# jhauret/vibravox

Hardware: AMD Instinct MI355X
Metric: EBEN train-step audio-seconds/sec (gen+disc) (higher is better)
Workload: dtype bf16

## Files before the change

### vibravox_amd/csrc/tap3.h

```cpp
#pragma once
#include "common.h"

namespace eben {

typedef unsigned u32x4 __attribute__((ext_vector_type(4)));

struct Tap3Args {
  const float* x; const float* xmask; const u32x4* wp; const int* tab;
  const float* bias; const float* res; const float* emask; float* y;
  int B, G, Cg, Mg, Cx, Cy, Lx, Ly;
  int S, OS, dstep, J0, mode, off0, nt, nph;
  int ps_pad, ps_k, ps_d, ps_kstep;
  int reflect, accumulate, in_mode;
  int res_rows, em_seg, em_map[4];
  const float* fm_sums; float fm_gs;
  float in_slope, out_slope, res_slope, emask_slope;
  int CI_T, CI_B, CP, ncc, PLEN, CSTRIDE, nxb;
  unsigned s_magic;
  int ntt, nmt, tab_phase;
  long long w_tile, w_phase;
  const u32x4* xh; const u32x4* xl;
  uint2* yh; uint2* yl;
  const uint2* eh; const uint2* el;
  const unsigned* ec;
  int CBx, CBy, bl_ref_off, bl_pad;
  int pr_S, pr_cbg, pr_Ly, pr_order;
  unsigned xq, xr;
  unsigned m_nph, m_ntt, m_B, m_nmt;
  int id_fast, pg_n;
  int big_XT, big_PPT, big_tiles;
  unsigned m_cstride, m_plen;
  struct PG { int J, off0, minoff, nt, oo, span; unsigned span_magic; int pad; } pg[8];
};

struct Tap3Plan {
  int ok;
  int mode, G, Cg, Mg, S, OS, dstep, kstep, nph, J, Lx, Ly, Cx, Cy, off0, nt, ps_pad;
  int FM, BM, BN, WCHU;
  int dense;
  int npw, npx, KSC;
  int CI_T, CI_B, CP, ncc, PLEN, CSTRIDE, nxbuf, XRB;
  int nmt, ntt, NCH, tab_phase;
  long long w_tile, w_phase, tab_off_floats;
  size_t packed_floats, lds_bytes;
  int big, WM, WN, TM, TN, RING, XT, PPT, xbuf_stride;
};

int tap4_launch(const Tap3Plan& p, const Tap3Args& a, hipStream_t st);

}
```

### vibravox_amd/csrc/tapconv3.hip

```cpp
#include "common.h"
#include "tap3.h"

#include <cstdlib>

namespace eben {

typedef float f32x16 __attribute__((ext_vector_type(16)));
typedef float f32x2 __attribute__((ext_vector_type(2)));
typedef __bf16 bf16x8 __attribute__((ext_vector_type(8)));
typedef __bf16 bf16x2 __attribute__((ext_vector_type(2)));

__device__ __forceinline__ unsigned pack_bf16(float a, float b) {
  const f32x2 v = {a, b};
  return __builtin_bit_cast(unsigned, __builtin_convertvector(v, bf16x2));
}

#ifndef EBEN_T3_KSC
#define EBEN_T3_KSC 4
#endif
#ifndef EBEN_T3_DBG
#define EBEN_T3_DBG 0
#endif
#if EBEN_T3_DBG & 512
constexpr int T3_STAMP_ROWS = 65536;
// ... 1059 lines not shown
  const int wave = __builtin_amdgcn_readfirstlane(tid >> 6);
  const int k = P.k;
  const int NCP = P.ncc * P.CP;
  int item = blockIdx.x;
  const int col = item % NCP; item /= NCP;
  const int fm = item % P.FM; item /= P.FM;
  const int mt = item % P.nmt;
  const int g = item / P.nmt;
  const int cc = col / P.CP, cp = col - cc * P.CP;
  const int m0 = mt * P.BM + fm * 32;
  const int c0 = cc * P.CI_T + 16 * cp;
  const int nrow = P.Mg - m0 < 32 ? P.Mg - m0 : 32;
  const int nch = P.Cg - c0 < 16 ? P.Cg - c0 : 16;
  const int RS = (P.mode == 0 ? 16 : 32) * k | 1;
  if (nrow > 0 && nch > 0) {
    const int nlines = P.mode == 0 ? nrow : nch;
    const int run = (P.mode == 0 ? nch : nrow) * k;
    for (int ln = wave; ln < nlines; ln += 4) {
      const long long src = P.mode == 0 ? ((long long)(g * P.Cout_g + m0 + ln) * P.Cin_g + c0) * k
                                        : ((long long)(g * P.Cout_g + c0 + ln) * P.Cin_g + m0) * k;
      const float sc = P.scale ? P.scale[g * P.Cout_g + (P.mode == 0 ? m0 : c0) + ln] : 1.f;
      for (int i = lane; i < run; i += 64) p3c[ln * RS + i] = P.w[src + i] * sc;
    }
  }
  __syncthreads();
  const int r = lane & 31, h = lane >> 5;
  const bool row_ok = r < nrow;
  u32x4* img = reinterpret_cast<u32x4*>(P.wp);
  const long long tile = (long long)g * P.nmt + mt;
  const bool last_col = col == NCP - 1;
  for (int ph = 0; ph < P.nph; ++ph) {
    int qJ, qk0;
    if (ph < 8) { qJ = P.pg[ph].J; qk0 = P.pg[ph].k0; }
    else { const PhaseGeom q = phase_geom(P.mode, ph, P.J0, P.off0, P.nt, P.dstep, P.OS, P.ps_pad, P.k, P.d, P.kstep, P.Ly); qJ = q.J; qk0 = q.k0; }
    const int KS_CC = qJ * P.CP, KS_all = P.ncc * KS_CC;
    const long long base = (long long)ph * P.w_phase + tile * P.w_tile;
    for (int j = wave; j < qJ; j += 4) {
      const int tap = P.mode == 0 ? j : qk0 + j * P.kstep;
      const int s = cc * KS_CC + j * P.CP + cp;
      const int ch = s / P.KSC, ks = s - ch * P.KSC;
      float v[8];
#pragma unroll
      for (int u = 0; u < 8; ++u) {
        const int c = 8 * h + u;
        const bool ok = row_ok && c < nch && tap < k;
        const int idx = P.mode == 0 ? r * RS + c * k + tap : c * RS + r * k + tap;
        v[u] = ok ? p3c[idx] : 0.f;
      }
      for (int piece = 0; piece < P.NPW; ++piece) {
        u32x4 o;
        o[0] = pack_bf16(v[0], v[1]); o[1] = pack_bf16(v[2], v[3]); o[2] = pack_bf16(v[4], v[5]); o[3] = pack_bf16(v[6], v[7]);
        img[base + (long long)ch * P.WCHU + ((ks * P.NPW + piece) * P.FM + fm) * 64 + lane] = o;
#pragma unroll
        for (int u = 0; u < 4; ++u) {
          v[2 * u] -= __builtin_bit_cast(float, o[u] << 16);
          v[2 * u + 1] -= __builtin_bit_cast(float, o[u] & 0xffff0000u);
        }
      }
    }
    if (last_col) {
      for (int s = KS_all + wave; s < P.NCH * P.KSC; s += 4) {
        const int ch = s / P.KSC, ks = s - ch * P.KSC;
        for (int piece = 0; piece < P.NPW; ++piece)
          img[base + (long long)ch * P.WCHU + ((ks * P.NPW + piece) * P.FM + fm) * 64 + lane] = u32x4{0u, 0u, 0u, 0u};
      }
    }
  }
}

__device__ __forceinline__ void pack3_tables(const Pack3Args& P) {
  const int tabs = P.tab_phase * P.nph;
  for (int r = threadIdx.x; r < tabs; r += 256) {
    const int ph = r / P.tab_phase;
    const int s = r - ph * P.tab_phase;
    const PhaseGeom q = phase_geom(P.mode, ph, P.J0, P.off0, P.nt, P.dstep, P.OS, P.ps_pad, P.k, P.d, P.kstep, P.Ly);
    const int KS_CC = q.J * P.CP;
    int o = 0;
    if (q.J > 0 && s < P.ncc * KS_CC) {
      const int cc = s / KS_CC, rem = s - cc * KS_CC;
      const int j = rem / P.CP, cp = rem - j * P.CP;
      const int rel = q.off0 + j * P.dstep - q.minoff;
      const int dd = rel / P.S, pp = rel - dd * P.S;
      o = (P.nxbuf > 1 ? (cc % P.nxbuf) * P.xbuf_stride : 0) + 2 * cp * P.CSTRIDE + pp * P.PLEN + dd;
    }
    reinterpret_cast<int*>(P.wp)[P.wunits * 4 + r] = o;
  }
}

__global__ __launch_bounds__(256) void pack3_kernel(const Pack3Args P) { pack3_body(P, blockIdx.x, gridDim.x); }

constexpr int PACK3_MULTI = 16;
struct Pack3Table {
  int n;
  unsigned first[PACK3_MULTI + 1];
  Pack3Args job[PACK3_MULTI];
};
__global__ __launch_bounds__(256) void pack3_multi_kernel(const Pack3Table T) {
  int j = 0;
#pragma unroll 1
  while (j + 1 < T.n && blockIdx.x >= T.first[j + 1]) ++j;
  pack3_body(T.job[j], blockIdx.x - T.first[j], T.first[j + 1] - T.first[j]);
}

template <int FM, int XRB, bool IM, int NPW = 1, int NPX = 1, bool BL = false>
static int launch3_im(const Tap3Args& a, int nblocks, size_t lds, hipStream_t st) {
  static LdsAttrOnce attr_once;
  auto kern = tap3_kernel<FM, XRB, IM, NPW, NPX, BL>;
  {
    const hipError_t e = lds_attr_once(attr_once, reinterpret_cast<const void*>(kern));
    if (e != hipSuccess) return hip_fail(e, "hipFuncSetAttribute(tap3)");
  }
  hipLaunchKernelGGL(kern, dim3(nblocks), dim3(256), lds, st, a);
  EBEN_CHECK_LAUNCH("tap3_kernel");
  return EBEN_OK;
}
template <int FM, int XRB>
static int launch3_cfg(const Tap3Args& a, int nblocks, size_t lds, int npw, int npx, hipStream_t st) {
  if (a.xh) {
    if (a.in_mode || npw != npx || npw > 2) return fail(EBEN_EUNSUPPORTED, "tap3: bundle layout with %d / %d operand pieces", npw, npx);
    if (npw == 2) return launch3_im<FM, XRB, false, 2, 2, true>(a, nblocks, lds, st);
    return launch3_im<FM, XRB, false, 1, 1, true>(a, nblocks, lds, st);
  }
  if (npx > 1) {
    if (a.in_mode) return fail(EBEN_EUNSUPPORTED, "tap3: split operand with a mask on load");
    if (npw == 1) return launch3_im<FM, XRB, false, 1, 2>(a, nblocks, lds, st);
    if (npw == 2) return launch3_im<FM, XRB, false, 2, 2>(a, nblocks, lds, st);
    return launch3_im<FM, XRB, false, 3, 3>(a, nblocks, lds, st);
  }
  return a.in_mode ? launch3_im<FM, XRB, true>(a, nblocks, lds, st) : launch3_im<FM, XRB, false>(a, nblocks, lds, st);
}

int tap3_applicable(const Canon& c, int dir) {
  Tap3Plan p;
  make_plan3(c, dir, &p);
  return p.ok;
}

int tap3_is_big(const Canon& c, int dir) {
  Tap3Plan p;
  make_plan3(c, dir, &p);
  return p.ok && p.big;
}

size_t tap3_packed_floats(const Canon& c, int dir) {
  Tap3Plan p;
  make_plan3(c, dir, &p);
  return p.ok ? p.packed_floats : 0;
}

static int tap3_pack_args(const Canon& c, int dir, const float* w, const float* scale, float* wp, Pack3Args* out, unsigned* blocks_out) {
  Tap3Plan p;
  make_plan3(c, dir, &p);
  if (!p.ok) return fail(EBEN_EUNSUPPORTED, "tap3_pack on a layer the bf16 kernel does not cover");
  Pack3Args a;
  a.w = w; a.scale = scale; a.wp = wp;
  a.G = p.G; a.Cg = p.Cg; a.Mg = p.Mg; a.nmt = p.nmt; a.BM = p.BM; a.FM = p.FM; a.WCHU = p.WCHU;
  a.CI_T = p.CI_T; a.CI_B = p.CI_B; a.CP = p.CP; a.ncc = p.ncc; a.NCH = p.NCH; a.nph = p.nph; a.tab_phase = p.tab_phase;
  a.mode = p.mode; a.J0 = p.J; a.off0 = p.off0; a.nt = p.nt; a.dstep = p.dstep; a.OS = p.OS; a.S = p.S; a.ps_pad = p.ps_pad;
  a.k = c.k; a.d = c.d; a.kstep = p.kstep; a.Ly = p.Ly;
  a.Cin_g = c.Cin / c.g; a.Cout_g = c.Cout / c.g; a.PLEN = p.PLEN; a.CSTRIDE = p.CSTRIDE; a.nxbuf = p.nxbuf; a.dense = p.dense;
  a.NPW = p.npw; a.KSC = p.KSC; a.xbuf_stride = p.xbuf_stride;
  a.w_tile = p.w_tile; a.w_phase = p.w_phase; a.wunits = p.w_phase * p.nph;
  long long blocks = (a.wunits + (long long)p.tab_phase * p.nph + 255) / 256;
  if (blocks > 8192) blocks = 8192;
  if (blocks < 1) blocks = 1;
  {
    const long long nmax = a.wunits + (long long)p.tab_phase * p.nph;
    if (nmax >= (1 << 24)) return fail(EBEN_EUNSUPPORTED, "tap3_pack: an image of %lld units is beyond the pack kernel's unit arithmetic", nmax);
    auto magic = [](long long d) { return d <= 1 ? 0u : (unsigned)((0x100000000ull + (unsigned long long)d - 1) / (unsigned long long)d); };
    a.r_wphase = 1.0f / (float)a.w_phase; a.r_wtile = 1.0f / (float)a.w_tile; a.m_nmt = magic(p.nmt); a.r_wchu = 1.0f / (float)p.WCHU; a.m_fm = magic(p.FM);
    a.m_npw = magic(p.npw); a.m_cp = magic(p.CP); a.m_coutg = magic(c.Cout / c.g);
    for (int ph = 0; ph < 8; ++ph) {
      a.pg[ph].J = 0; a.pg[ph].k0 = 0; a.pg[ph].m_kscc = 0; a.pg[ph].pad = 0;
      if (ph >= p.nph) continue;
      const PhaseGeom q = phase_geom(p.mode, ph, p.J, p.off0, p.nt, p.dstep, p.OS, p.ps_pad, c.k, c.d, p.kstep, p.Ly);
      a.pg[ph].J = q.J; a.pg[ph].k0 = q.k0; a.pg[ph].m_kscc = magic((long long)q.J * p.CP);
    }
  }
  *out = a;
  *blocks_out = (unsigned)blocks;
  return EBEN_OK;
}

static int tap3_pack_coalesced(const Pack3Args& a, hipStream_t st, int* rc) {
  static const long long min_w = getenv("EBEN_PACK3C_MIN") ? atoll(getenv("EBEN_PACK3C_MIN")) : 200000;
  *rc = EBEN_OK;
  const long long weights = (long long)a.G * a.Cout_g * a.Cin_g * a.k;
  const size_t lds = sizeof(float) * (size_t)(a.mode == 0 ? 32 : 16) * (size_t)(((a.mode == 0 ? 16 : 32) * a.k) | 1);
  if (min_w <= 0 || a.dense || weights < min_w || lds > 150 * 1024 || a.nph > 8) return 0;
  static LdsAttrOnce attr_once;
  {
    const hipError_t e = lds_attr_once(attr_once, reinterpret_cast<const void*>(pack3c_kernel));
    if (e != hipSuccess) { *rc = hip_fail(e, "hipFuncSetAttribute(pack3c)"); return 1; }
  }
  const long long items = (long long)a.G * a.nmt * a.FM * a.ncc * a.CP;
  hipLaunchKernelGGL(pack3c_kernel, dim3((unsigned)items), dim3(256), lds, st, a);
  hipError_t e = hipGetLastError();
  if (e != hipSuccess) *rc = hip_fail(e, "pack3c_kernel");
  return 1;
}

int tap3_pack(const Canon& c, int dir, const float* w, const float* scale, float* wp, hipStream_t st) {
  Pack3Args a;
  unsigned blocks;
  int rc = tap3_pack_args(c, dir, w, scale, wp, &a, &blocks);
  if (rc) return rc;
  if (tap3_pack_coalesced(a, st, &rc)) return rc;
  hipLaunchKernelGGL(pack3_kernel, dim3(blocks), dim3(256), 0, st, a);
  EBEN_CHECK_LAUNCH("pack3_kernel");
  return EBEN_OK;
}

int tap3_pack_multi(const Canon* cs, const int* dirs, const float* const* ws, const float* const* scales, float* const* wps, int n, hipStream_t st) {
  for (int base = 0; base < n; base += PACK3_MULTI) {
    Pack3Table T;
    T.n = n - base < PACK3_MULTI ? n - base : PACK3_MULTI;
    T.first[0] = 0;
    for (int j = 0; j < T.n; ++j) {
      unsigned blocks;
      int rc = tap3_pack_args(cs[base + j], dirs[base + j], ws[base + j], scales[base + j], wps[base + j], &T.job[j], &blocks);
      if (rc) return rc;
      if (tap3_pack_coalesced(T.job[j], st, &rc)) {
        if (rc) return rc;
        T.job[j].wunits = 0; T.job[j].tab_phase = 0;
        blocks = 1;
      }
      { static const unsigned cap = getenv("EBEN_PACK3_CAP") ? (unsigned)atoi(getenv("EBEN_PACK3_CAP")) : 512u; if (blocks > cap) blocks = cap; }
      T.first[j + 1] = T.first[j] + blocks;
    }
    hipLaunchKernelGGL(pack3_multi_kernel, dim3(T.first[T.n]), dim3(256), 0, st, T);
    EBEN_CHECK_LAUNCH("pack3_multi_kernel");
  }
  return EBEN_OK;
}

int tap3_launch(const Canon& c, int dir, const TapIO& io, int reflect, hipStream_t st) {
  Tap3Plan p;
  make_plan3(c, dir, &p);
  if (!p.ok) return fail(EBEN_EUNSUPPORTED, "tap3_launch on a layer the bf16 kernel does not cover");
  Tap3Args a;
  a.x = io.x; a.xmask = io.in_mode ? io.xmask : io.x; a.in_mode = io.in_mode; a.wp = reinterpret_cast<const u32x4*>(io.wp); a.tab = reinterpret_cast<const int*>(io.wp + p.tab_off_floats);
  a.bias = io.bias; a.res = io.res; a.emask = io.emask; a.y = io.y;
  a.xh = a.xl = nullptr; a.yh = a.yl = nullptr; a.eh = a.el = nullptr; a.ec = nullptr; a.CBx = a.CBy = a.bl_ref_off = a.bl_pad = 0;
  a.pr_S = a.pr_cbg = a.pr_Ly = a.pr_order = 0;
  if (c.bl) {
    if (!io.xh || !io.yh || (p.npx > 1 && !io.xl)) return fail(EBEN_EINVAL, "tap3: null bundle-layout plane");
    a.xh = static_cast<const u32x4*>(io.xh); a.xl = static_cast<const u32x4*>(io.xl);
    a.yh = static_cast<uint2*>(io.yh); a.yl = static_cast<uint2*>(io.yl);
    a.eh = static_cast<const uint2*>(io.eh); a.el = static_cast<const uint2*>(io.el); a.ec = static_cast<const unsigned*>(io.ec);
    a.CBx = p.Cx >> 3; a.CBy = p.Cy >> 3; a.bl_ref_off = io.bl_ref_off;
    a.x = nullptr; a.xmask = nullptr;
    if (io.pr_S > 0) {
      if (dir != 0 || p.S != 1 || p.nph != 1) return fail(EBEN_EINVAL, "tap3: phases-as-rows output on a launch that is not a stride-1 gather");
      a.pr_S = io.pr_S; a.pr_cbg = io.pr_cbg; a.pr_Ly = io.pr_Ly; a.CBy = io.pr_CBy; a.pr_order = io.pr_order;
      if (p.big && io.pr_order != 1) return fail(EBEN_EINVAL, "tap3: phases-as-rows order %d on a launch plan that is tap4's", io.pr_order);
      if (io.pr_order == 1 && ((io.pr_S != 4 && io.pr_S != 2) || (io.pr_S == 4 && (p.Mg & 31)) || (p.Mg & 15) || !c.bl || (p.big && io.pr_S != 4)))
        return fail(EBEN_EINVAL, "tap3: bundle-major phases as rows need stride 4 (whole 32-row tiles) or 2 (whole 16-row bundles)");
    }
  } else if (io.xh) {
    return fail(EBEN_EINVAL, "tap3: bundle-layout planes on a descriptor without EBEN_LAYOUT_BL");
  }
  a.B = c.B; a.G = p.G; a.Cg = p.Cg; a.Mg = p.Mg; a.Cx = p.Cx; a.Cy = p.Cy; a.Lx = p.Lx; a.Ly = p.Ly;
  a.S = p.S; a.OS = p.OS; a.dstep = p.dstep; a.J0 = p.J; a.mode = p.mode; a.off0 = p.off0; a.nt = p.nt; a.nph = p.nph;
  a.ps_pad = p.ps_pad; a.ps_k = c.k; a.ps_d = c.d; a.ps_kstep = p.kstep;
  a.reflect = reflect; a.accumulate = io.accumulate;
  a.res_rows = io.res_rows; a.em_seg = io.em_seg; a.fm_sums = io.fm_sums; a.fm_gs = io.fm_gs;
  for (int i = 0; i < 4; ++i) a.em_map[i] = io.em_map[i];
  a.in_slope = io.in_slope; a.out_slope = io.out_slope; a.res_slope = io.res_slope; a.emask_slope = io.emask_slope;
  a.CI_T = p.CI_T; a.CI_B = p.CI_B; a.CP = p.CP; a.ncc = p.ncc; a.PLEN = p.PLEN; a.CSTRIDE = p.CSTRIDE; a.nxb = p.nxbuf;
  a.s_magic = p.S > 1 ? (unsigned)((0x100000000ull + p.S - 1) / p.S) : 0u;
  a.ntt = p.ntt; a.nmt = p.nmt; a.tab_phase = p.tab_phase;
  a.w_tile = p.w_tile; a.w_phase = p.w_phase;
  const long long nb = (long long)p.ntt * c.B * p.nph * p.nmt * p.G;
  if (nb <= 0 || nb > 0x7fffffffLL) return fail(EBEN_EINVAL, "tap3 grid of %lld blocks", nb);
  a.big_XT = p.XT; a.big_PPT = p.PPT; a.big_tiles = (int)nb;
  a.m_cstride = (unsigned)((0x100000000ull + (unsigned)p.CSTRIDE - 1) / (unsigned)p.CSTRIDE);
  a.m_plen = p.S > 1 ? (unsigned)((0x100000000ull + (unsigned)p.PLEN - 1) / (unsigned)p.PLEN) : 0u;
  a.xq = (unsigned)(nb / 8); a.xr = (unsigned)(nb % 8);
  {
    auto magic = [](int d) { return (unsigned)((0x100000000ull + (unsigned)d - 1) / (unsigned)d); };
    int dmax = p.nph > p.ntt ? p.nph : p.ntt;
    if (c.B > dmax) dmax = c.B;
    if (p.nmt > dmax) dmax = p.nmt;
    a.id_fast = nb * dmax < 0x100000000LL ? 1 : 0;
    a.m_nph = magic(p.nph); a.m_ntt = magic(p.ntt); a.m_B = magic(c.B); a.m_nmt = magic(p.nmt);
    if (p.nph == 1) a.m_nph = 0;
    if (p.ntt == 1) a.m_ntt = 0;
    if (c.B == 1) a.m_B = 0;
    if (p.nmt == 1) a.m_nmt = 0;
    a.pg_n = p.nph <= 8 ? p.nph : 0;
    const int ad = p.dstep >= 0 ? p.dstep : -p.dstep;
    for (int ph = 0; ph < a.pg_n; ++ph) {
      const PhaseGeom q = phase_geom(p.mode, ph, p.J, p.off0, p.nt, p.dstep, p.OS, p.ps_pad, c.k, c.d, p.kstep, p.Ly);
      a.pg[ph].J = q.J; a.pg[ph].off0 = q.off0; a.pg[ph].minoff = q.minoff; a.pg[ph].nt = q.nt; a.pg[ph].oo = q.oo;
      a.pg[ph].span = q.J > 0 ? (p.BN - 1) * p.S + (q.J - 1) * ad + 1 : 0;
      a.pg[ph].span_magic = a.pg[ph].span > 0 ? magic(a.pg[ph].span) : 0u;
      a.pg[ph].pad = 0;
    }
  }
  if (p.big) {
    if (p.nph > 8) return fail(EBEN_EUNSUPPORTED, "tap4: more than 8 output phases");
    return tap4_launch(p, a, st);
  }
#define EBEN_T3_CASE(FMV)                                                          \
  switch (p.XRB) {                                                                 \
    case 2: return launch3_cfg<FMV, 2>(a, (int)nb, p.lds_bytes, p.npw, p.npx, st);               \
    case 3: return launch3_cfg<FMV, 3>(a, (int)nb, p.lds_bytes, p.npw, p.npx, st);               \
    default: return launch3_cfg<FMV, 5>(a, (int)nb, p.lds_bytes, p.npw, p.npx, st);              \
  }
  switch (p.FM) {
    case 1: EBEN_T3_CASE(1)
    case 2: EBEN_T3_CASE(2)
    case 3: EBEN_T3_CASE(3)
    default: EBEN_T3_CASE(4)
  }
#undef EBEN_T3_CASE
}

}

#if EBEN_T3_DBG & 512
extern "C" __attribute__((visibility("default"))) int eben_debug_t3_stamps(unsigned long long* out, int rows) {
  if (rows > eben::T3_STAMP_ROWS) rows = eben::T3_STAMP_ROWS;
  if (out && hipMemcpyFromSymbol(out, HIP_SYMBOL(eben::t3_stamp), (size_t)rows * 128) != hipSuccess) return 1;
  if (!out) {
    void* p = nullptr;
    if (hipGetSymbolAddress(&p, HIP_SYMBOL(eben::t3_stamp)) != hipSuccess || hipMemset(p, 0, sizeof(unsigned long long) * eben::T3_STAMP_ROWS * 16) != hipSuccess) return 1;
  }
  return 0;
}
#endif
```

Baseline: 7538.

## Add specialized thin-channel tap-conv kernel for bf16 hi/lo forward and backward cases

Result: faster. 7702, median of 6 (+2.2%).

```diff
diff --git a/vibravox_amd/csrc/tap3.h b/vibravox_amd/csrc/tap3.h
--- a/vibravox_amd/csrc/tap3.h
+++ b/vibravox_amd/csrc/tap3.h
@@ -47,5 +47,6 @@
 };
 
 int tap4_launch(const Tap3Plan& p, const Tap3Args& a, hipStream_t st);
+int thin_bl_launch(const Tap3Plan& p, const Tap3Args& a, int reflect, int nblocks, hipStream_t st, int* rc);
 
 }
diff --git a/vibravox_amd/csrc/tapconv3.hip b/vibravox_amd/csrc/tapconv3.hip
--- a/vibravox_amd/csrc/tapconv3.hip
+++ b/vibravox_amd/csrc/tapconv3.hip
@@ -1385,6 +1385,10 @@
     if (p.nph > 8) return fail(EBEN_EUNSUPPORTED, "tap4: more than 8 output phases");
     return tap4_launch(p, a, st);
   }
+  {
+    int rc = EBEN_OK;
+    if (thin_bl_launch(p, a, reflect, (int)nb, st, &rc)) return rc;
+  }
 #define EBEN_T3_CASE(FMV)                                                          \
   switch (p.XRB) {                                                                 \
     case 2: return launch3_cfg<FMV, 2>(a, (int)nb, p.lds_bytes, p.npw, p.npx, st);               \
diff --git a/vibravox_amd/csrc/thin_bl.hip b/vibravox_amd/csrc/thin_bl.hip
--- /dev/null
+++ b/vibravox_amd/csrc/thin_bl.hip
@@ -0,0 +1,550 @@
+#include "common.h"
+#include "tap3.h"
+
+#include <cstdlib>
+
+namespace eben {
+namespace thin {
+
+typedef float f32x16 __attribute__((ext_vector_type(16)));
+typedef float f32x2 __attribute__((ext_vector_type(2)));
+typedef __bf16 bf16x8 __attribute__((ext_vector_type(8)));
+typedef __bf16 bf16x2 __attribute__((ext_vector_type(2)));
+
+__device__ __forceinline__ unsigned pack_bf16(float a, float b) {
+  const f32x2 v = {a, b};
+  return __builtin_bit_cast(unsigned, __builtin_convertvector(v, bf16x2));
+}
+template <int N> __device__ __forceinline__ void wait_vm() {
+  static_assert(N >= 0 && N < 64, "vmcnt is a 6-bit count");
+  __builtin_amdgcn_s_waitcnt((N & 15) | ((N >> 4) << 14) | 0x70);
+}
+__device__ u32x4 zero_unit = {0u, 0u, 0u, 0u};
+
+enum { FWD = 0, DX_PR = 1, DX_PS = 2 };
+
+constexpr int ksc_of(int np) { return np == 1 ? 4 : 2; }
+constexpr int RING = 2;
+
+template <int FM, int NP, int DIR, int S>
+__global__ __launch_bounds__(256, NP >= 2 ? 1 : 2) void thin_bl_kernel(const Tap3Args P) {
+  constexpr int NT = 256, BN = 128, BM = FM * 32, KSC = ksc_of(NP);
+  constexpr int WCHU = KSC * NP * FM * 64;
+  constexpr int WU = (WCHU + NT - 1) / NT;
+  constexpr int CS = DIR == FWD ? S : 1;
+  constexpr bool DMA_X = CS == 1;
+  constexpr bool DX = DIR != FWD;
+  static_assert(WCHU % 64 == 0, "weight chunk must split into whole wave pieces");
+
+  extern __shared__ __attribute__((aligned(16))) u32x4 smem_thin[];
+  u32x4* Ws = smem_thin;
+  u32x4* Xs = smem_thin + RING * WCHU;
+
+  const int tid = threadIdx.x;
+  const int lane = tid & 63;
+  const int wn = __builtin_amdgcn_readfirstlane(tid >> 6);
+
+  unsigned id;
+  {
+    const unsigned bid = blockIdx.x, xcd = bid & 7u, idx = bid >> 3;
+    id = (xcd < P.xr ? xcd * (P.xq + 1) : P.xr * (P.xq + 1) + (xcd - P.xr) * P.xq) + idx;
+  }
+  int ph = 0, tt, b, mt, g;
+  if (P.id_fast) {
+    unsigned qd;
+    if constexpr (DIR == DX_PS) { qd = P.m_nph ? __umulhi(id, P.m_nph) : id; ph = (int)(id - qd * (unsigned)P.nph); id = qd; }
+    qd = P.m_ntt ? __umulhi(id, P.m_ntt) : id; tt = (int)(id - qd * (unsigned)P.ntt); id = qd;
+    qd = P.m_B ? __umulhi(id, P.m_B) : id; b = (int)(id - qd * (unsigned)P.B); id = qd;
+    qd = P.m_nmt ? __umulhi(id, P.m_nmt) : id; mt = (int)(id - qd * (unsigned)P.nmt); g = (int)qd;
+  } else {
+    if constexpr (DIR == DX_PS) { ph = id % P.nph; id /= P.nph; }
+    tt = id % P.ntt; id /= P.ntt;
+    b = id % P.B; id /= P.B;
+    mt = id % P.nmt;
+    g = id / P.nmt;
+  }
+  ph = __builtin_amdgcn_readfirstlane(ph); tt = __builtin_amdgcn_readfirstlane(tt); b = __builtin_amdgcn_readfirstlane(b);
+  mt = __builtin_amdgcn_readfirstlane(mt); g = __builtin_amdgcn_readfirstlane(g);
+  const int t0 = tt * BN, m0 = mt * BM;
+
+  const int J = P.pg[ph].J, nt = P.pg[ph].nt, oo = DIR == DX_PS ? P.pg[ph].oo : 0, minoff = P.pg[ph].minoff, span = P.pg[ph].span;
+  const unsigned span_magic = P.pg[ph].span_magic;
+  if (t0 >= nt) return;
+  const int KS = J * P.CP;
+  const int nch = (KS + KSC - 1) / KSC;
+  const int q0 = t0 * CS + minoff;
+  const int xtot = P.CI_B * span;
+  const int XBUF = P.CI_B * P.CSTRIDE;
+  const int LOU = NP > 1 ? XBUF + 1 : 0;
+
+  const u32x4* wsrc = P.wp + (long long)ph * P.w_phase + ((long long)g * P.nmt + mt) * P.w_tile;
+  typedef const __attribute__((address_space(4))) int* ctab_t;
+  ctab_t tab = (ctab_t)(P.tab + (long long)ph * P.tab_phase);
+
+  f32x16 acc[FM];
+#pragma unroll
+  for (int i = 0; i < FM; ++i)
+#pragma unroll
+    for (int r = 0; r < 16; ++r) acc[i][r] = 0.f;
+
+  const int CgB = P.Cg >> 3;
+  const long long xrowB = ((long long)b * P.CBx + (long long)g * CgB) * P.Lx;
+  const bool inside = q0 >= 0 && q0 + span <= P.Lx;
+
+  auto issue_w = [&](int ch) {
+    const u32x4* src = wsrc + (long long)ch * WCHU;
+    u32x4* dst = Ws + (ch % RING) * WCHU;
+#pragma unroll
+    for (int u = 0; u < WU; ++u) {
+      int idx = u * NT + tid;
+      if (WCHU % NT != 0 && idx >= WCHU) idx -= NT;
+      __builtin_amdgcn_global_load_lds((const __attribute__((address_space(1))) void*)(src + idx),
+                                       (__attribute__((address_space(3))) void*)(dst + (idx & ~63)), 16, 0, 0);
+    }
+  };
+
+  int eb = b;
+  if constexpr (DX) {
+    eb = P.em_seg > 0 ? P.em_map[(int)(b >= P.em_seg) + (int)(b >= 2 * P.em_seg) + (int)(b >= 3 * P.em_seg)] * P.em_seg +
+                            (b - ((int)(b >= P.em_seg) + (int)(b >= 2 * P.em_seg) + (int)(b >= 3 * P.em_seg)) * P.em_seg) : b;
+  }
+  float* Bs = reinterpret_cast<float*>(Xs + NP * (XBUF + 1));
+  float fk1 = 0.f, fk2 = 0.f;
+  const bool fmr = DX && P.fm_sums != nullptr && P.res_rows > 0 && b < P.res_rows;
+  if constexpr (!DX) {
+    if (tid < BM) {
+      const int m = m0 + tid;
+      Bs[tid] = P.bias ? P.bias[(long long)g * P.Mg + (m < P.Mg ? m : P.Mg - 1)] : 0.f;
+    }
+  } else if (fmr) {
+    typedef const __attribute__((address_space(4))) float* cf_t;
+    const float s1 = ((cf_t)P.fm_sums)[0], s2 = ((cf_t)P.fm_sums)[1];
+    fk1 = P.fm_gs / s2; fk2 = P.fm_gs * s1 / (s2 * s2);
+  }
+  if (nch > 0) {
+    issue_w(0);
+    if constexpr (DMA_X) {
+      const int ppr = (span + 63) >> 6;
+      int bb = 0, pr = __builtin_amdgcn_readfirstlane(tid >> 6);
+      while (pr >= ppr) { pr -= ppr; ++bb; }
+      while (bb < P.CI_B) {
+        const int r = pr * 64 + lane;
+        const int qq = q0 + r;
+        const bool in = qq >= 0 && qq < P.Lx && bb < CgB;
+        const long long idx = xrowB + (long long)(bb < CgB ? bb : 0) * P.Lx + (in ? qq : 0);
+        u32x4* d = Xs + bb * P.CSTRIDE + pr * 64;
+        if (r < span) {
+          __builtin_amdgcn_global_load_lds((const __attribute__((address_space(1))) void*)(in ? P.xh + idx : &zero_unit),
+                                           (__attribute__((address_space(3))) void*)d, 16, 0, 0);
+          if constexpr (NP > 1)
+            __builtin_amdgcn_global_load_lds((const __attribute__((address_space(1))) void*)(in ? P.xl + idx : &zero_unit),
+                                             (__attribute__((address_space(3))) void*)(d + LOU), 16, 0, 0);
+        }
+        pr += NT / 64;
+        while (pr >= ppr) { pr -= ppr; ++bb; }
+      }
+    } else {
+      struct Round { u32x4 w[2][NP]; int sl[2], ok[2]; };
+      auto pro_load = [&](int base, Round& R) {
+#pragma unroll
+        for (int u = 0; u < 2; ++u) {
+          const int i = base + tid + u * NT;
+          const int bb = (int)__umulhi((unsigned)i, span_magic);
+          const int r = i - bb * span;
+          int qq = q0 + (i < xtot ? r : 0), ok = 1;
+          if (!inside) {
+            ok = (int)(qq >= 0) & (int)(qq < P.Lx);
+            qq = ok ? qq : 0;
+          }
+          ok &= (int)(i < xtot);
+          const int c0 = i < xtot ? bb : 0;
+          ok &= (int)(c0 < CgB);
+          const long long idx = xrowB + (long long)(c0 < CgB ? c0 : 0) * P.Lx + qq;
+          R.w[u][0] = P.xh[idx];
+          if constexpr (NP > 1) R.w[u][1] = P.xl[idx];
+          R.ok[u] = ok;
+          const int d = r / CS, p = r - d * CS;
+          R.sl[u] = i < xtot ? bb * P.CSTRIDE + p * P.PLEN + d : -1;
+        }
+      };
+      auto pro_store = [&](Round& R) {
+#pragma unroll
+        for (int u = 0; u < 2; ++u)
+          if (R.sl[u] >= 0) {
+#pragma unroll
+            for (int q = 0; q < NP; ++q) Xs[R.sl[u] + q * LOU] = R.ok[u] ? R.w[u][q] : u32x4{0u, 0u, 0u, 0u};
+          }
+      };
+      Round ra, rb;
+      if (xtot > 0) pro_load(0, ra);
+      for (int base = 0; base < xtot; base += 4 * NT) {
+        const bool second = base + 2 * NT < xtot;
+        if (second) pro_load(base + 2 * NT, rb);
+        pro_store(ra);
+        if (second) {
+          if (base + 4 * NT < xtot) pro_load(base + 4 * NT, ra);
+          pro_store(rb);
+        }
+      }
+    }
+  }
+  __syncthreads();
+  constexpr bool PREF = DIR == DX_PS && FM <= 2;
+  uint2 pah[PREF ? FM : 1][4];
+  if constexpr (PREF) {
+    if (P.eh != nullptr) {
+      const int tq = t0 + wn * 32 + (lane & 31);
+      const unsigned loffq = (((unsigned)(tq < nt ? tq : nt - 1) * (unsigned)P.OS + (unsigned)oo) * 2u + (unsigned)(lane >> 5)) * 8u;
+      const long long Lrowq = (long long)P.Ly * 16;
+      const char* ehq = reinterpret_cast<const char*>(P.eh) + (long long)eb * P.CBy * Lrowq + ((long long)((g * P.Mg + m0) >> 3)) * Lrowq;
+      const int quadsq = (P.Mg - m0 + 7) >> 3;
+#pragma unroll
+      for (int i = 0; i < FM; ++i)
+#pragma unroll
+        for (int r4 = 0; r4 < 4; ++r4) {
+          const int q = 4 * i + r4;
+          pah[i][r4] = *reinterpret_cast<const uint2*>(ehq + (long long)(q < quadsq ? q : 0) * Lrowq + loffq);
+        }
+    }
+  }
+
+  const int lanebase = (lane >> 5) * P.CSTRIDE + wn * 32 + (lane & 31);
+  int te[KSC];
+#pragma unroll
+  for (int ks = 0; ks < KSC; ++ks) te[ks] = nch > 0 ? tab[ks] : 0;
+  constexpr int H = KSC >= 2 ? KSC / 2 : 1, H2 = KSC - H;
+  u32x4 bvA[H][NP], aA[H][NP][FM], bvB[H2 > 0 ? H2 : 1][NP], aB[H2 > 0 ? H2 : 1][NP][FM];
+  auto mma = [&](const u32x4 (&bq)[NP], const u32x4 (&aq)[NP][FM]) {
+#pragma unroll
+    for (int lvl = NP - 1; lvl >= 0; --lvl)
+#pragma unroll
+      for (int qw = 0; qw < NP; ++qw) {
+        const int qx = lvl - qw;
+        if (qx < 0 || qx >= NP) continue;
+#pragma unroll
+        for (int i = 0; i < FM; ++i)
+          acc[i] = __builtin_amdgcn_mfma_f32_32x32x16_bf16(__builtin_bit_cast(bf16x8, aq[qw][i]), __builtin_bit_cast(bf16x8, bq[qx]), acc[i], 0, 0, 0);
+      }
+  };
+  for (int ch = 0; ch < nch; ++ch) {
+    int tn[KSC];
+#pragma unroll
+    for (int ks = 0; ks < KSC; ++ks) tn[ks] = tab[(ch + 1 < nch ? ch + 1 : ch) * KSC + ks];
+    if (ch + 1 < nch) issue_w(ch + 1);
+    const u32x4* wb = Ws + (ch % RING) * WCHU + lane;
+    const u32x4* xb = Xs + lanebase;
+    auto rd = [&](int ks, u32x4 (&bq)[NP], u32x4 (&aq)[NP][FM]) {
+#pragma unroll
+      for (int q = 0; q < NP; ++q) bq[q] = xb[te[ks] + q * LOU];
+#pragma unroll
+      for (int q = 0; q < NP; ++q)
+#pragma unroll
+        for (int i = 0; i < FM; ++i) aq[q][i] = wb[((ks * NP + q) * FM + i) * 64];
+    };
+#pragma unroll
+    for (int h = 0; h < H; ++h) rd(h, bvA[h], aA[h]);
+    __builtin_amdgcn_sched_barrier(0);
+    if (ch > 0) {
+#pragma unroll
+      for (int h = 0; h < H2; ++h) mma(bvB[h], aB[h]);
+    }
+    __builtin_amdgcn_sched_barrier(0);
+#pragma unroll
+    for (int h = 0; h < H2; ++h) rd(H + h, bvB[h], aB[h]);
+    __builtin_amdgcn_sched_barrier(0);
+#pragma unroll
+    for (int h = 0; h < H; ++h) mma(bvA[h], aA[h]);
+    __builtin_amdgcn_sched_barrier(0);
+#pragma unroll
+    for (int ks = 0; ks < KSC; ++ks) te[ks] = tn[ks];
+    wait_vm<0>();
+    __builtin_amdgcn_s_barrier();
+  }
+  if (nch > 0) {
+#pragma unroll
+    for (int h = 0; h < H2; ++h) mma(bvB[h], aB[h]);
+  }
+
+  const int t = t0 + wn * 32 + (lane & 31);
+  if (t >= nt) return;
+  const int hb = lane >> 5;
+  auto unpack = [](uint2 w, float (&f)[4]) {
+    f[0] = __builtin_bit_cast(float, w.x << 16); f[1] = __builtin_bit_cast(float, w.x & 0xffff0000u);
+    f[2] = __builtin_bit_cast(float, w.y << 16); f[3] = __builtin_bit_cast(float, w.y & 0xffff0000u);
+  };
+  const bool masked = DX && P.eh != nullptr;
+  const bool fmc = fmr && masked && P.ec != nullptr;
+
+  if constexpr (DIR == DX_PR) {
+    constexpr bool s4 = S == 4;
+    static_assert(S == 2 || S == 4, "phases as rows at stride 2 or 4");
+    const int tile0i = m0 >> 5;
+    const long long LrowP = (long long)P.pr_Ly * 16;
+    const long long tileP = (long long)(g * P.pr_cbg) * LrowP;
+    const char* ehp = reinterpret_cast<const char*>(P.eh) + (long long)eb * P.CBy * LrowP + tileP;
+    const char* elp = reinterpret_cast<const char*>(P.el) + (long long)eb * P.CBy * LrowP + tileP;
+    const char* rhp = reinterpret_cast<const char*>(P.eh) + (long long)(b + P.bl_ref_off) * P.CBy * LrowP + tileP;
+    const char* rlp = reinterpret_cast<const char*>(P.el) + (long long)(b + P.bl_ref_off) * P.CBy * LrowP + tileP;
+    char* yhp = reinterpret_cast<char*>(P.yh) + (long long)b * P.CBy * LrowP + tileP;
+    char* ylp = reinterpret_cast<char*>(P.yl) + (long long)b * P.CBy * LrowP + tileP;
+    const int pos0 = s4 ? 4 * t + 2 * hb : 2 * t;
+    const bool lv0 = pos0 < P.pr_Ly, lv1 = pos0 + 1 < P.pr_Ly;
+    const unsigned poff = (unsigned)(lv0 ? pos0 : 0) * 16u;
+    auto bund = [&](int i) { return s4 ? tile0i + i : 2 * (tile0i + i) + hb; };
+    auto swap32 = [](unsigned& x, unsigned& y) {
+      const auto r = __builtin_amdgcn_permlane32_swap(x, y, false, false);
+      x = r[0]; y = r[1];
+    };
+    auto to_halves = [&](const u32x4 (&U)[2], uint2 (&Hh)[4]) {
+#pragma unroll
+      for (int j = 0; j < 2; ++j) {
+        unsigned x0 = U[j][0], x1 = U[j][1], y0 = U[j][2], y1 = U[j][3];
+        swap32(x0, y0); swap32(x1, y1);
+        Hh[j].x = x0; Hh[j].y = x1; Hh[2 + j].x = y0; Hh[2 + j].y = y1;
+      }
+    };
+    auto to_units = [&](const uint2 (&Hh)[4], u32x4 (&U)[2]) {
+#pragma unroll
+      for (int j = 0; j < 2; ++j) {
+        unsigned x0 = Hh[j].x, x1 = Hh[j].y, y0 = Hh[2 + j].x, y1 = Hh[2 + j].y;
+        swap32(x0, y0); swap32(x1, y1);
+        U[j] = u32x4{x0, x1, y0, y1};
+      }
+    };
+    auto ldu = [&](const char* base, int i, u32x4 (&U)[2]) {
+      const int bd = bund(i);
+      const char* q = base + (long long)(bd < P.pr_cbg ? bd : 0) * LrowP + poff;
+      U[0] = *reinterpret_cast<const u32x4*>(q);
+      U[1] = *reinterpret_cast<const u32x4*>(q + (lv1 ? 16 : 0));
+    };
+    auto stu = [&](int i, const uint2 (&Hh)[4], char* base) {
+      u32x4 U[2];
+      to_units(Hh, U);
+      const int bd = bund(i);
+      char* q = base + (long long)bd * LrowP + poff;
+      if (bd >= P.pr_cbg) return;
+      if (lv0) *reinterpret_cast<u32x4*>(q) = U[0];
+      if (lv1) *reinterpret_cast<u32x4*>(q + 16) = U[1];
+    };
+    const int tiles = (P.Mg - m0 + 31) >> 5;
+    const char* ecp = reinterpret_cast<const char*>(P.ec) + (((long long)eb * P.CBy * LrowP + tileP) >> 1);
+    u32x4 AU[FM][2];
+    if (masked && (!fmr || fmc)) {
+#pragma unroll
+      for (int i = 0; i < FM; ++i) ldu(ehp, i < tiles ? i : 0, AU[i]);
+    }
+#pragma unroll
+    for (int i = 0; i < FM; ++i) {
+      if (i >= tiles) continue;
+      uint2 AH[4], AL[4], RH[4], RL[4], OH[4], OL[4];
+      unsigned CW[4] = {0u, 0u, 0u, 0u};
+      if (masked && (!fmr || fmc)) {
+        to_halves(AU[i], AH);
+        if (fmc) {
+          const int bd = bund(i);
+          const char* q = ecp + (((long long)(bd < P.pr_cbg ? bd : 0) * LrowP + poff) >> 1);
+          const uint2 c0 = *reinterpret_cast<const uint2*>(q);
+          const uint2 c1 = *reinterpret_cast<const uint2*>(q + (lv1 ? 8 : 0));
+          unsigned x0 = c0.x, y0 = c0.y, x1 = c1.x, y1 = c1.y;
+          swap32(x0, y0); swap32(x1, y1);
+          CW[0] = x0; CW[2] = y0; CW[1] = x1; CW[3] = y1;
+        }
+      } else if (masked) {
+        u32x4 A2[2], L2[2], RH2[2], RL2[2];
+        ldu(ehp, i, A2); ldu(elp, i, L2); ldu(rhp, i, RH2); ldu(rlp, i, RL2);
+        to_halves(A2, AH); to_halves(L2, AL); to_halves(RH2, RH); to_halves(RL2, RL);
+      }
+#pragma unroll
+      for (int r4 = 0; r4 < 4; ++r4) {
+        float v[4], a0[4];
+#pragma unroll
+        for (int e = 0; e < 4; ++e) v[e] = acc[i][4 * r4 + e];
+        if (masked) {
+          unpack(AH[r4], a0);
+          if (fmc) {
+#pragma unroll
+            for (int e = 0; e < 4; ++e) {
+              const unsigned c = CW[r4] >> (8 * e);
+              v[e] += fk1 * (float)((int)(c & 3u) - 1) - fk2 * (float)((int)((c >> 2) & 3u) - 1);
+            }
+          } else if (fmr) {
+            float a1[4], r0[4], r1[4];
+            unpack(AL[r4], a1); unpack(RH[r4], r0); unpack(RL[r4], r1);
+#pragma unroll
+            for (int e = 0; e < 4; ++e) {
+              const float av = a0[e] + a1[e], dv = av - (r0[e] + r1[e]);
+              v[e] += fk1 * (float)((dv > 0.f) - (dv < 0.f)) - fk2 * (float)((av > 0.f) - (av < 0.f));
+            }
+          }
+#pragma unroll
+          for (int e = 0; e < 4; ++e) v[e] *= dlrelu(a0[e], P.emask_slope);
+        } else {
+#pragma unroll
+          for (int e = 0; e < 4; ++e) v[e] = lrelu(v[e], P.out_slope);
+        }
+        OH[r4].x = pack_bf16(v[0], v[1]); OH[r4].y = pack_bf16(v[2], v[3]);
+        float hf[4];
+        unpack(OH[r4], hf);
+        OL[r4].x = pack_bf16(v[0] - hf[0], v[1] - hf[1]); OL[r4].y = pack_bf16(v[2] - hf[2], v[3] - hf[3]);
+      }
+      stu(i, OH, yhp);
+      if (P.yl) stu(i, OL, ylp);
+    }
+    return;
+  } else {
+    const unsigned loff = (((unsigned)t * (unsigned)P.OS + (unsigned)oo) * 2u + (unsigned)hb) * 8u;
+    const long long Lrow = (long long)P.Ly * 16;
+    const long long tile0 = ((long long)((g * P.Mg + m0) >> 3)) * Lrow;
+    char* yhb = reinterpret_cast<char*>(P.yh) + (long long)b * P.CBy * Lrow + tile0;
+    char* ylb = reinterpret_cast<char*>(P.yl) + (long long)b * P.CBy * Lrow + tile0;
+    const int quads = (P.Mg - m0 + 7) >> 3;
+    if constexpr (DIR == FWD) {
+#pragma unroll
+      for (int i = 0; i < FM; ++i) {
+        float bz[4][4];
+#pragma unroll
+        for (int r4 = 0; r4 < 4; ++r4) {
+          const float4 bq = *reinterpret_cast<const float4*>(Bs + i * 32 + 8 * r4 + 4 * hb);
+          bz[r4][0] = bq.x; bz[r4][1] = bq.y; bz[r4][2] = bq.z; bz[r4][3] = bq.w;
+        }
+#pragma unroll
+        for (int r4 = 0; r4 < 4; ++r4) {
+          const int q = 4 * i + r4;
+          if (q >= quads) continue;
+          const long long row = (long long)q * Lrow;
+          float v[4];
+#pragma unroll
+          for (int e = 0; e < 4; ++e) v[e] = lrelu(acc[i][4 * r4 + e] + bz[r4][e], P.out_slope);
+          uint2 h;
+          h.x = pack_bf16(v[0], v[1]); h.y = pack_bf16(v[2], v[3]);
+          *reinterpret_cast<uint2*>(yhb + row + loff) = h;
+          if (P.yl) {
+            float hf[4];
+            unpack(h, hf);
+            uint2 l;
+            l.x = pack_bf16(v[0] - hf[0], v[1] - hf[1]); l.y = pack_bf16(v[2] - hf[2], v[3] - hf[3]);
+            *reinterpret_cast<uint2*>(ylb + row + loff) = l;
+          }
+        }
+      }
+    } else {
+      const char* ehb = reinterpret_cast<const char*>(P.eh) + (long long)eb * P.CBy * Lrow + tile0;
+      const char* elb = reinterpret_cast<const char*>(P.el) + (long long)eb * P.CBy * Lrow + tile0;
+      const char* rhb = reinterpret_cast<const char*>(P.eh) + (long long)(b + P.bl_ref_off) * P.CBy * Lrow + tile0;
+      const char* rlb = reinterpret_cast<const char*>(P.el) + (long long)(b + P.bl_ref_off) * P.CBy * Lrow + tile0;
+      const char* ecb = reinterpret_cast<const char*>(P.ec) + (((long long)eb * P.CBy * Lrow + tile0) >> 1);
+      auto ld2 = [&](const char* base, long long row) { return *reinterpret_cast<const uint2*>(base + row + loff); };
+#pragma unroll
+      for (int i = 0; i < FM; ++i) {
+        uint2 ah[4], al[4], rh[4], rl[4];
+        unsigned cw[4];
+#pragma unroll
+        for (int r4 = 0; r4 < 4; ++r4) {
+          const int q = 4 * i + r4;
+          const long long row = (long long)(q < quads ? q : 0) * Lrow;
+          if (masked) {
+            if constexpr (PREF) ah[r4] = pah[i][r4];
+            else ah[r4] = ld2(ehb, row);
+            if (fmc) cw[r4] = *reinterpret_cast<const unsigned*>(ecb + ((row + (long long)loff) >> 1));
+            else if (fmr) { al[r4] = ld2(elb, row); rh[r4] = ld2(rhb, row); rl[r4] = ld2(rlb, row); }
+          }
+        }
+#pragma unroll
+        for (int r4 = 0; r4 < 4; ++r4) {
+          const int q = 4 * i + r4;
+          if (q >= quads) continue;
+          const long long row = (long long)q * Lrow;
+          float v[4], a0[4];
+#pragma unroll
+          for (int e = 0; e < 4; ++e) v[e] = acc[i][4 * r4 + e] + 0.f;
+          if (masked) {
+            unpack(ah[r4], a0);
+            if (fmc) {
+#pragma unroll
+              for (int e = 0; e < 4; ++e) {
+                const unsigned c = cw[r4] >> (8 * e);
+                v[e] += fk1 * (float)((int)(c & 3u) - 1) - fk2 * (float)((int)((c >> 2) & 3u) - 1);
+              }
+            } else if (fmr) {
+              float a1[4], r0[4], r1[4];
+              unpack(al[r4], a1); unpack(rh[r4], r0); unpack(rl[r4], r1);
+#pragma unroll
+              for (int e = 0; e < 4; ++e) {
+                const float av = a0[e] + a1[e], dv = av - (r0[e] + r1[e]);
+                v[e] += fk1 * (float)((dv > 0.f) - (dv < 0.f)) - fk2 * (float)((av > 0.f) - (av < 0.f));
+              }
+            }
+#pragma unroll
+            for (int e = 0; e < 4; ++e) v[e] *= dlrelu(a0[e], P.emask_slope);
+          } else {
+#pragma unroll
+            for (int e = 0; e < 4; ++e) v[e] = lrelu(v[e], P.out_slope);
+          }
+          uint2 h;
+          h.x = pack_bf16(v[0], v[1]); h.y = pack_bf16(v[2], v[3]);
+          *reinterpret_cast<uint2*>(yhb + row + loff) = h;
+          if (P.yl) {
+            float hf[4];
+            unpack(h, hf);
+            uint2 l;
+            l.x = pack_bf16(v[0] - hf[0], v[1] - hf[1]); l.y = pack_bf16(v[2] - hf[2], v[3] - hf[3]);
+            *reinterpret_cast<uint2*>(ylb + row + loff) = l;
+          }
+        }
+      }
+    }
+  }
+}
+
+template <int FM, int NP, int DIR, int S>
+static int launch(const Tap3Args& a, int nblocks, size_t lds, hipStream_t st) {
+  static LdsAttrOnce attr_once;
+  auto kern = thin_bl_kernel<FM, NP, DIR, S>;
+  {
+    const hipError_t e = lds_attr_once(attr_once, reinterpret_cast<const void*>(kern));
+    if (e != hipSuccess) return hip_fail(e, "hipFuncSetAttribute(thin_bl)");
+  }
+  hipLaunchKernelGGL(kern, dim3(nblocks), dim3(256), lds, st, a);
+  EBEN_CHECK_LAUNCH("thin_bl_kernel");
+  return EBEN_OK;
+}
+
+template <int NP, int DIR, int S>
+static int launch_fm(int FM, const Tap3Args& a, int nblocks, size_t lds, hipStream_t st) {
+  switch (FM) {
+    case 1: return launch<1, NP, DIR, S>(a, nblocks, lds, st);
+    case 2: return launch<2, NP, DIR, S>(a, nblocks, lds, st);
+    case 3: return launch<3, NP, DIR, S>(a, nblocks, lds, st);
+    default: return launch<4, NP, DIR, S>(a, nblocks, lds, st);
+  }
+}
+
+}
+
+int thin_bl_launch(const Tap3Plan& p, const Tap3Args& a, int reflect, int nblocks, hipStream_t st, int* rc) {
+  static const int enabled = getenv("EBEN_THIN_BL") ? atoi(getenv("EBEN_THIN_BL")) : 1;
+  if (!enabled || !a.xh || p.big || reflect || a.in_mode || p.npw != p.npx || p.npw > 2) return 0;
+  if (p.ncc != 1 || p.nxbuf != 1 || p.nph > 8 || p.FM < 1 || p.FM > 4 || p.BN != 128) return 0;
+  if (p.KSC != thin::ksc_of(p.npw) || p.WCHU != p.KSC * p.npw * p.FM * 64) return 0;
+  if (p.lds_bytes != (size_t)thin::RING * p.WCHU * 16 + ((size_t)p.CI_B * p.CSTRIDE * 16 + 16) * p.npx + (size_t)p.BM * 4) return 0;
+  if (p.Cg > 128 || p.Mg > 256) return 0;
+  const size_t lds = p.lds_bytes;
+  if (p.mode == 0 && a.pr_S == 0) {
+    if (a.eh || a.res || a.accumulate || p.nph != 1) return 0;
+    if (p.S == 2 && p.npw == 2) { *rc = thin::launch_fm<2, thin::FWD, 2>(p.FM, a, nblocks, lds, st); return 1; }
+    if (p.S == 4 && p.npw == 1) { *rc = thin::launch_fm<1, thin::FWD, 4>(p.FM, a, nblocks, lds, st); return 1; }
+    return 0;
+  }
+  if (p.npw != 1 || a.bias || a.res || a.accumulate) return 0;
+  if (p.mode == 0) {
+    if (a.pr_order != 1 || p.S != 1 || p.nph != 1) return 0;
+    if (a.pr_S == 2) { *rc = thin::launch_fm<1, thin::DX_PR, 2>(p.FM, a, nblocks, lds, st); return 1; }
+    if (a.pr_S == 4) { *rc = thin::launch_fm<1, thin::DX_PR, 4>(p.FM, a, nblocks, lds, st); return 1; }
+    return 0;
+  }
+  if (p.S != 1 || p.OS != 2 || p.nph != 2) return 0;
+  *rc = thin::launch_fm<1, thin::DX_PS, 1>(p.FM, a, nblocks, lds, st);
+  return 1;
+}
+
+}
```
